# royshil/SfM-Toy-Library

Measured on NVIDIA H100. Metric: BA residual+Jacobian evals/sec, higher is better.
Workload: dtype f64

## Files before the change

sfm-toy-library_b200/csrc/ba.cu:

```cuda
#include "common.cuh"
#include "ba_math.cuh"
#include "chol.cuh"
#include <algorithm>
#include <chrono>
#include <cmath>
#include <cstdlib>

namespace {

constexpr int PT_THREADS = 128;
constexpr int PTB = 18;
constexpr int CAM_THREADS = 128;

struct LMState {
    double radius, decrease_factor, x_cost, x_norm, gmax, initial_cost;
    double msg_a, msg_b;
    double last_rho;
    int cur, iter, invalid_steps, new_point;
    int status;
    int termination_type;
    int num_successful, num_unsuccessful;
    int passes;
};
enum { LM_RUNNING = 0, LM_EVAL_FAILED = 1, LM_GRADIENT_TOL = 2, LM_MAX_TIME = 3, LM_MAX_ITER = 4, LM_MIN_RADIUS = 5, LM_INVALID_STEPS = 6,
       LM_PARAMETER_TOL = 7, LM_FUNCTION_TOL = 8 };

struct BAView {
    int nc, np, nobs, maxk;
    const LMState* st;
    double* cf2[2]; double* pts2[2]; CamDerived* camd2[2];
    const float2* obs_xy; const int32_t* obs_cam; const int32_t* pt_off;
    const int32_t* cm_off; const float2* cm_xy; const int32_t* cm_pt;
    const double* cams; const double* pts; const double* focal;
    const CamDerived* camd;
    const double* scale_cf; const double* scale_pt;
    double* ptblk;
    double* Zbuf;
    double* Sblk; double* Scf; double* Sff; double* rhs; double* gcf; double* dcf; double* sums;
    unsigned long long* gmax_pt_bits;
    int* fail;
    double min_diag, max_diag;
    double* part4;
    unsigned* counters;
};

__device__ __forceinline__ bool last_block_sum4(double* __restrict__ part4, unsigned* __restrict__ counter, const double (&mine)[4], double (&out)[4]) {
    __shared__ bool last_s;
    if (threadIdx.x == 0) {
#pragma unroll
        for (int q = 0; q < 4; ++q) part4[4 * (size_t)blockIdx.x + q] = mine[q];
        __threadfence();
        last_s = atomicInc(counter, gridDim.x - 1) == gridDim.x - 1;
    }
    __syncthreads();
    if (!last_s || threadIdx.x >= 32) return false;
    __threadfence();
    double acc[4] = {0.0, 0.0, 0.0, 0.0};
    for (unsigned b = threadIdx.x; b < gridDim.x; b += 32) {
#pragma unroll
        for (int q = 0; q < 4; ++q) acc[q] += __ldcg(part4 + 4 * (size_t)b + q);
    }
#pragma unroll
    for (int q = 0; q < 4; ++q) {
#pragma unroll
        for (int o = 16; o > 0; o >>= 1) acc[q] += __shfl_xor_sync(0xffffffffu, acc[q], o);
        out[q] = acc[q];
    }
    return true;
}

struct LMX { const double* focal; const double* pts; const CamDerived* camd; bool run; };
__device__ __forceinline__ LMX lm_x(const BAView& v) {
    LMX x; x.focal = v.focal; x.pts = v.pts; x.camd = v.camd; x.run = true;
    if (v.st) {
        x.run = v.st->status == LM_RUNNING;
        const int cur = v.st->cur;
        x.focal = v.cf2[cur] + 6 * v.nc; x.pts = v.pts2[cur]; x.camd = v.camd2[cur];
    }
    return x;
}

__device__ __forceinline__ void red_add(double* p, double v) {
    asm volatile("red.global.add.f64 [%0], %1;" ::"l"(p), "d"(v) : "memory");
}
__device__ __forceinline__ double clampd(double v, double lo, double hi) { return fmin(fmax(v, lo), hi); }
__device__ __forceinline__ size_t blk_index(int i, int j, int nb) {
    return (size_t)i * nb - (size_t)i * (i - 1) / 2 + (j - i);
}

template <int G>
__device__ __forceinline__ double group_sum(double v, unsigned mask) {
#pragma unroll
    for (int o = G / 2; o > 0; o >>= 1) v += __shfl_xor_sync(mask, v, o);
    return v;
}
__device__ __forceinline__ double warp_sum(double v) {
#pragma unroll
    for (int o = 16; o > 0; o >>= 1) v += __shfl_xor_sync(0xffffffffu, v, o);
    return v;
}
__device__ __forceinline__ double warp_max(double v) {
#pragma unroll
    for (int o = 16; o > 0; o >>= 1) v = fmax(v, __shfl_xor_sync(0xffffffffu, v, o));
    return v;
}

struct ObsJ { double r[2], Jc[12], Jp[6], Jf[2]; };
__device__ __forceinline__ void eval_scaled(const CamDerived& d, const double* X, double f, float2 xy,
                                            const double* sc , const double* sp , double sf, ObsJ& o) {
    obs_eval(d, X, f, (double)xy.x, (double)xy.y, o.r, o.Jc, o.Jp, o.Jf);
#pragma unroll
    for (int a = 0; a < 6; ++a) { o.Jc[a] *= sc[a]; o.Jc[6 + a] *= sc[a]; }
#pragma unroll
    for (int a = 0; a < 3; ++a) { o.Jp[a] *= sp[a]; o.Jp[3 + a] *= sp[a]; }
    o.Jf[0] *= sf; o.Jf[1] *= sf;
}

__global__ void cam_derive_kernel(const double* __restrict__ cams, int nc, CamDerived* __restrict__ out) {
    const int c = blockIdx.x * blockDim.x + threadIdx.x;
    if (c < nc) { CamDerived d; cam_derive(cams + 6 * c, d); out[c] = d; }
}

template <int G>
__global__ void __launch_bounds__(PT_THREADS) ba_point_norm_kernel(BAView v, double* __restrict__ scale_pt_out) {
    const int lane = threadIdx.x & 31, gl = lane % G;
    const unsigned gmask = G == 32 ? 0xffffffffu : (((1u << G) - 1u) << ((lane / G) * G));
    const int groups_per_block = PT_THREADS / G;
    const double f = *v.focal;
    for (int p = blockIdx.x * groups_per_block + threadIdx.x / G; p < v.np; p += gridDim.x * groups_per_block) {
        const int o0 = v.pt_off[p], k = v.pt_off[p + 1] - o0;
        const double X[3] = {v.pts[3 * p], v.pts[3 * p + 1], v.pts[3 * p + 2]};
        double n0 = 0, n1 = 0, n2 = 0;
        for (int j = gl; j < k; j += G) {
            const int o = o0 + j;
            double r[2], Jc[12], Jp[6], Jf[2];
            const float2 xy = v.obs_xy[o];
            obs_eval(v.camd[v.obs_cam[o]], X, f, (double)xy.x, (double)xy.y, r, Jc, Jp, Jf);
            n0 += Jp[0] * Jp[0] + Jp[3] * Jp[3]; n1 += Jp[1] * Jp[1] + Jp[4] * Jp[4]; n2 += Jp[2] * Jp[2] + Jp[5] * Jp[5];
        }
        n0 = group_sum<G>(n0, gmask); n1 = group_sum<G>(n1, gmask); n2 = group_sum<G>(n2, gmask);
        if (gl == 0) {
            scale_pt_out[3 * p] = 1.0 / (1.0 + sqrt(n0)); scale_pt_out[3 * p + 1] = 1.0 / (1.0 + sqrt(n1));
            scale_pt_out[3 * p + 2] = 1.0 / (1.0 + sqrt(n2));
        }
    }
}

__global__ void __launch_bounds__(CAM_THREADS) ba_camera_norm_kernel(BAView v, double* __restrict__ colnorm_cf) {
    const int c = blockIdx.y;
    const int begin = v.cm_off[c], end = v.cm_off[c + 1];
    const CamDerived d = v.camd[c];
    const double f = *v.focal;
    double n[7] = {0, 0, 0, 0, 0, 0, 0};
    for (int i = begin + blockIdx.x * CAM_THREADS + threadIdx.x; i < end; i += gridDim.x * CAM_THREADS) {
        const int p = v.cm_pt[i];
        const double X[3] = {v.pts[3 * p], v.pts[3 * p + 1], v.pts[3 * p + 2]};
        double r[2], Jc[12], Jp[6], Jf[2];
        const float2 xy = v.cm_xy[i];
        obs_eval(d, X, f, (double)xy.x, (double)xy.y, r, Jc, Jp, Jf);
#pragma unroll
        for (int a = 0; a < 6; ++a) n[a] += Jc[a] * Jc[a] + Jc[6 + a] * Jc[6 + a];
        n[6] += Jf[0] * Jf[0] + Jf[1] * Jf[1];
    }
    __shared__ double red[CAM_THREADS / 32][7];
#pragma unroll
    for (int a = 0; a < 7; ++a) { const double s = warp_sum(n[a]); if ((threadIdx.x & 31) == 0) red[threadIdx.x >> 5][a] = s; }
    __syncthreads();
    if (threadIdx.x < 7) {
        double s = 0;
        for (int w = 0; w < CAM_THREADS / 32; ++w) s += red[w][threadIdx.x];
        if (s != 0.0) red_add(threadIdx.x < 6 ? colnorm_cf + 6 * c + threadIdx.x : colnorm_cf + 6 * v.nc, s);
    }
}

__global__ void scale_from_norm_kernel(const double* __restrict__ colnorm, int n, double* __restrict__ scale) {
    const int i = blockIdx.x * blockDim.x + threadIdx.x;
    if (i < n) scale[i] = 1.0 / (1.0 + sqrt(colnorm[i]));
}
__global__ void fill_kernel(double* __restrict__ p, size_t n, double v) {
    const size_t i = (size_t)blockIdx.x * blockDim.x + threadIdx.x;
    if (i < n) p[i] = v;
}

template <int G, bool GATHER>
__global__ void __launch_bounds__(PT_THREADS, 3) ba_point_kernel(BAView v, double inv_radius) {
    const LMX x = lm_x(v);
    if (!x.run) return;
    if (v.st) inv_radius = 1.0 / v.st->radius;
    extern __shared__ __align__(16) unsigned char smem_raw[];
    __shared__ __align__(16) double zstage[GATHER ? PT_THREADS / 32 : 1][GATHER ? 32 * 18 : 2];
    constexpr int GB = PT_THREADS / G, GW = 32 / G;
    const int maxk = v.maxk;
    double* Zall = reinterpret_cast<double*>(smem_raw);
    int* camall = reinterpret_cast<int*>(Zall + (size_t)GB * maxk * 18);
    unsigned short* pair_tab = reinterpret_cast<unsigned short*>(camall + GB * maxk);
    if (!GATHER) {
        for (int j = 1 + threadIdx.x / 32; j < maxk; j += PT_THREADS / 32)
            for (int i = threadIdx.x & 31; i < j; i += 32) pair_tab[j * (j - 1) / 2 + i] = (unsigned short)(i | (j << 8));
        __syncthreads();
    }

    const int lane = threadIdx.x & 31, warp = threadIdx.x >> 5, gl = lane % G, gi = lane / G;
    const unsigned gmask = G == 32 ? 0xffffffffu : (((1u << G) - 1u) << (gi * G));
    const int group_in_block = warp * GW + gi;
    double* Zg = GATHER ? nullptr : Zall + (size_t)group_in_block * maxk * 18;
    int* camg = GATHER ? nullptr : camall + group_in_block * maxk;
    const double f = *x.focal, sf = v.scale_cf[6 * v.nc];
    const int nb = v.nc;

    double acc_cost = 0, acc_xn = 0, acc_sff = 0, acc_rf = 0, acc_gmax = 0;
    const int np_round = (v.np + GB - 1) / GB * GB;
    for (int base = blockIdx.x * GB; base < np_round; base += gridDim.x * GB) {
        const int p = base + group_in_block;
        const bool active = p < v.np;
        int o0 = 0, k = 0;
        double X[3] = {0, 0, 0}, sp[3] = {1, 1, 1};
        {
            const int pn = p + gridDim.x * GB;
            if (pn < v.np && gl == 0) {
                const int on = v.pt_off[pn];
                asm volatile("prefetch.global.L2 [%0];" :: "l"(v.obs_cam + on)); asm volatile("prefetch.global.L2 [%0];" :: "l"(v.obs_xy + on));
                asm volatile("prefetch.global.L2 [%0];" :: "l"(x.pts + 3 * (size_t)pn)); asm volatile("prefetch.global.L2 [%0];" :: "l"(v.scale_pt + 3 * (size_t)pn));
            }
        }
        if (active) {
            o0 = v.pt_off[p]; k = v.pt_off[p + 1] - o0;
            X[0] = x.pts[3 * p]; X[1] = x.pts[3 * p + 1]; X[2] = x.pts[3 * p + 2];
            sp[0] = v.scale_pt[3 * p]; sp[1] = v.scale_pt[3 * p + 1]; sp[2] = v.scale_pt[3 * p + 2];
        }
        double U[6] = {0, 0, 0, 0, 0, 0}, g[3] = {0, 0, 0}, wf[3] = {0, 0, 0}, cost = 0;
        double Wreg[18];
        for (int j = gl; j < k; j += G) {
            const int o = o0 + j, c = v.obs_cam[o];
            ObsJ J;
            eval_scaled(x.camd[c], X, f, v.obs_xy[o], v.scale_cf + 6 * c, sp, sf, J);
            const double* e = J.Jp;
            U[0] += e[0] * e[0] + e[3] * e[3]; U[1] += e[0] * e[1] + e[3] * e[4]; U[2] += e[0] * e[2] + e[3] * e[5];
            U[3] += e[1] * e[1] + e[4] * e[4]; U[4] += e[1] * e[2] + e[4] * e[5]; U[5] += e[2] * e[2] + e[5] * e[5];
#pragma unroll
            for (int a = 0; a < 3; ++a) { g[a] += e[a] * J.r[0] + e[3 + a] * J.r[1]; wf[a] += e[a] * J.Jf[0] + e[3 + a] * J.Jf[1]; }
            cost += J.r[0] * J.r[0] + J.r[1] * J.r[1];
            if (GATHER && j == gl) {
#pragma unroll
                for (int a = 0; a < 6; ++a)
#pragma unroll
                    for (int b = 0; b < 3; ++b) Wreg[a * 3 + b] = J.Jc[a] * e[b] + J.Jc[6 + a] * e[3 + b];
            } else {
                double* W = GATHER ? v.Zbuf + (size_t)o * 18 : Zg + j * 18;
#pragma unroll
                for (int a = 0; a < 6; ++a)
#pragma unroll
                    for (int b = 0; b < 3; ++b) W[a * 3 + b] = J.Jc[a] * e[b] + J.Jc[6 + a] * e[3 + b];
            }
            if (!GATHER) camg[j] = c;
        }
#pragma unroll
        for (int a = 0; a < 6; ++a) U[a] = group_sum<G>(U[a], gmask);
#pragma unroll
        for (int a = 0; a < 3; ++a) { g[a] = group_sum<G>(g[a], gmask); wf[a] = group_sum<G>(wf[a], gmask); }
        cost = group_sum<G>(cost, gmask);

        const double udiag[3] = {U[0], U[3], U[5]};
        U[0] += clampd(U[0], v.min_diag, v.max_diag) * inv_radius;
        U[3] += clampd(U[3], v.min_diag, v.max_diag) * inv_radius;
        U[5] += clampd(U[5], v.min_diag, v.max_diag) * inv_radius;
        double M[6] = {0, 0, 0, 0, 0, 0};
        const bool ok = chol3_inverse(U, M);
        if (!ok) { M[0] = M[1] = M[2] = M[3] = M[4] = M[5] = 0.0; }
        const double zg[3] = {M[0] * g[0], M[1] * g[0] + M[2] * g[1], M[3] * g[0] + M[4] * g[1] + M[5] * g[2]};
        const double zf[3] = {M[0] * wf[0], M[1] * wf[0] + M[2] * wf[1], M[3] * wf[0] + M[4] * wf[1] + M[5] * wf[2]};
        if (active) {
            const double blk[PTB] = {M[0], M[1], M[2], M[3], M[4], M[5], zg[0], zg[1], zg[2], zf[0], zf[1], zf[2], g[0], g[1], g[2], udiag[0], udiag[1], udiag[2]};
#pragma unroll
            for (int q = 0; q < PTB; ++q) if ((q % G) == gl) v.ptblk[(size_t)p * PTB + q] = blk[q];
            if (gl == 0) {
                if (!ok && k > 0) atomicAdd(v.fail, 1);
                acc_cost += cost;
                acc_xn += X[0] * X[0] + X[1] * X[1] + X[2] * X[2];
                acc_sff += zf[0] * zf[0] + zf[1] * zf[1] + zf[2] * zf[2];
                acc_rf += zf[0] * zg[0] + zf[1] * zg[1] + zf[2] * zg[2];
                acc_gmax = fmax(acc_gmax, fmax(fabs(g[0] / sp[0]), fmax(fabs(g[1] / sp[1]), fabs(g[2] / sp[2]))));
            }
        }
        const bool stage = GATHER && v.maxk <= G;
        int o_first = 0, o_end = 0;
        if (stage) {
            const int p_first = base + warp * GW;
            o_first = p_first < v.np ? v.pt_off[p_first] : 0; o_end = p_first < v.np ? v.pt_off[min(p_first + GW, v.np)] : 0;
        }
        if (GATHER && gl < k) {
            double2* dst = stage ? reinterpret_cast<double2*>(zstage[warp] + (size_t)(o0 + gl - o_first) * 18)
                                 : reinterpret_cast<double2*>(v.Zbuf + (size_t)(o0 + gl) * 18);
#pragma unroll
            for (int a = 0; a < 6; a += 2) {
                double z[6];
#pragma unroll
                for (int h = 0; h < 2; ++h) {
                    const double w0 = Wreg[(a + h) * 3], w1 = Wreg[(a + h) * 3 + 1], w2 = Wreg[(a + h) * 3 + 2];
                    z[3 * h] = w0 * M[0]; z[3 * h + 1] = w0 * M[1] + w1 * M[2]; z[3 * h + 2] = w0 * M[3] + w1 * M[4] + w2 * M[5];
                }
                dst[a / 2 * 3] = make_double2(z[0], z[1]); dst[a / 2 * 3 + 1] = make_double2(z[2], z[3]); dst[a / 2 * 3 + 2] = make_double2(z[4], z[5]);
            }
        }
        if (stage) {
            __syncwarp();
            const double2* src = reinterpret_cast<const double2*>(zstage[warp]);
            double2* out = reinterpret_cast<double2*>(v.Zbuf + (size_t)o_first * 18);
            for (int i = lane; i < (o_end - o_first) * 9; i += 32) out[i] = src[i];
            __syncwarp();
        }
        for (int j = gl + (GATHER ? G : 0); j < k; j += G) {
            double* W = GATHER ? v.Zbuf + (size_t)(o0 + j) * 18 : Zg + j * 18;
#pragma unroll
            for (int a = 0; a < 6; ++a) {
                const double w0 = W[a * 3], w1 = W[a * 3 + 1], w2 = W[a * 3 + 2];
                W[a * 3] = w0 * M[0]; W[a * 3 + 1] = w0 * M[1] + w1 * M[2]; W[a * 3 + 2] = w0 * M[3] + w1 * M[4] + w2 * M[5];
            }
        }
        if (GATHER) continue;
        __syncwarp();
#pragma unroll 1
        for (int gs = 0; gs < GW; ++gs) {
            const int kk = __shfl_sync(0xffffffffu, k, gs * G);
            const double* Zs = Zall + (size_t)(warp * GW + gs) * maxk * 18;
            const int* cs = camall + (warp * GW + gs) * maxk;
            const int total = kk * (kk - 1) / 2 * 36;
            for (int e = lane; e < total; e += 32) {
                const int pr = e / 36, ab = e - pr * 36, a = ab / 6, b = ab - a * 6;
                const unsigned ij = pair_tab[pr];
                const int i = ij & 0xff, j = ij >> 8;
                const double* zi = Zs + i * 18 + a * 3; const double* zj = Zs + j * 18 + b * 3;
                const double val = zi[0] * zj[0] + zi[1] * zj[1] + zi[2] * zj[2];
                red_add(v.Sblk + blk_index(cs[i], cs[j], nb) * 36 + ab, -val);
            }
        }
        __syncwarp();
    }
    __shared__ double sred[PT_THREADS / 32][5];
    const double c0 = warp_sum(acc_cost), c1 = warp_sum(acc_xn), c2 = warp_sum(acc_sff), c3 = warp_sum(acc_rf), c4 = warp_max(acc_gmax);
    if (lane == 0) { sred[warp][0] = c0; sred[warp][1] = c1; sred[warp][2] = c2; sred[warp][3] = c3; sred[warp][4] = c4; }
    __syncthreads();
    double t[4] = {0, 0, 0, 0};
    if (threadIdx.x == 0) {
        double t4 = 0;
        for (int w = 0; w < PT_THREADS / 32; ++w) { t[0] += sred[w][0]; t[1] += sred[w][1]; t[2] += sred[w][2]; t[3] += sred[w][3]; t4 = fmax(t4, sred[w][4]); }
        atomicMax(v.gmax_pt_bits, (unsigned long long)__double_as_longlong(t4));
        if (!GATHER) {
            red_add(v.sums + 0, t[0]); red_add(v.sums + 1, t[1]);
            red_add(v.Sff, -t[2]); red_add(v.rhs + 6 * v.nc, -t[3]);
        }
    }
    if (GATHER) {
        double tot[4];
        if (last_block_sum4(v.part4, v.counters + 0, t, tot) && threadIdx.x == 0) {
            v.sums[0] = tot[0]; v.sums[1] = tot[1]; *v.Sff = -tot[2]; v.rhs[6 * v.nc] = -tot[3];
        }
    }
}

__device__ __forceinline__ void dmma_m8n8k4(double& c0, double& c1, double a, double b) {
    asm volatile("mma.sync.aligned.m8n8k4.row.col.f64.f64.f64.f64 {%0,%1}, {%2}, {%3}, {%0,%1};" : "+d"(c0), "+d"(c1) : "d"(a), "d"(b));
}

constexpr int CAM_REC = 64;
template <bool DET, bool NORM_ONLY>
__global__ void __launch_bounds__(CAM_THREADS) ba_camera_kernel(BAView v, int per_cta, double* __restrict__ cam_part) {
    const LMX x = lm_x(v);
    if (!x.run) return;
    const int start = blockIdx.x * per_cta, stop = min(v.nobs, start + per_cta);
    if (start >= stop) return;
    int c = 0;
    {
        int lo = 0, hi = v.nc - 1;
        while (lo < hi) { const int mid = (lo + hi + 1) >> 1; if (v.cm_off[mid] <= start) lo = mid; else hi = mid - 1; }
        c = lo;
    }
    const double f = *x.focal, sf = NORM_ONLY ? 1.0 : v.scale_cf[6 * v.nc];
    __shared__ double red[CAM_THREADS / 32][48];
    const int lane = threadIdx.x & 31, warp = threadIdx.x >> 5;
    for (; c < v.nc && v.cm_off[c] < stop; ++c) {
    const int begin = max(start, v.cm_off[c]), end = min(stop, v.cm_off[c + 1]);
    if (begin >= end) continue;
    const CamDerived d = x.camd[c];
    double sc[6];
#pragma unroll
    for (int a = 0; a < 6; ++a) sc[a] = NORM_ONLY ? 1.0 : v.scale_cf[6 * c + a];
    double A[21], Cf[6], R[6], Gd[6], D[6], ff = 0, gf = 0;
#pragma unroll
    for (int a = 0; a < 21; ++a) A[a] = 0;
#pragma unroll
    for (int a = 0; a < 6; ++a) { Cf[a] = 0; R[a] = 0; Gd[a] = 0; D[a] = 0; }
    for (int i = begin + threadIdx.x; i < end; i += CAM_THREADS) {
        const int p = v.cm_pt[i];
        const double X[3] = {x.pts[3 * p], x.pts[3 * p + 1], x.pts[3 * p + 2]};
        ObsJ J;
        if (NORM_ONLY) {
            const double one[3] = {1.0, 1.0, 1.0};
            eval_scaled(d, X, f, v.cm_xy[i], sc, one, 1.0, J);
            ff += J.Jf[0] * J.Jf[0] + J.Jf[1] * J.Jf[1];
#pragma unroll
            for (int a = 0; a < 6; ++a) D[a] += J.Jc[a] * J.Jc[a] + J.Jc[6 + a] * J.Jc[6 + a];
            continue;
        }
        const double sp[3] = {v.scale_pt[3 * p], v.scale_pt[3 * p + 1], v.scale_pt[3 * p + 2]};
        const double* pb = v.ptblk + (size_t)p * PTB;
        const double M[6] = {pb[0], pb[1], pb[2], pb[3], pb[4], pb[5]};
        const double zg[3] = {pb[6], pb[7], pb[8]}, zf[3] = {pb[9], pb[10], pb[11]};
        eval_scaled(d, X, f, v.cm_xy[i], sc, sp, sf, J);
        ff += J.Jf[0] * J.Jf[0] + J.Jf[1] * J.Jf[1];
        gf += J.Jf[0] * J.r[0] + J.Jf[1] * J.r[1];
        double Z[6][3];
#pragma unroll
        for (int a = 0; a < 6; ++a) {
            const double w0 = J.Jc[a] * J.Jp[0] + J.Jc[6 + a] * J.Jp[3], w1 = J.Jc[a] * J.Jp[1] + J.Jc[6 + a] * J.Jp[4],
                         w2 = J.Jc[a] * J.Jp[2] + J.Jc[6 + a] * J.Jp[5];
            Z[a][0] = w0 * M[0]; Z[a][1] = w0 * M[1] + w1 * M[2]; Z[a][2] = w0 * M[3] + w1 * M[4] + w2 * M[5];
            const double jr = J.Jc[a] * J.r[0] + J.Jc[6 + a] * J.r[1];
            Gd[a] += jr;
            R[a] += jr - (Z[a][0] * zg[0] + Z[a][1] * zg[1] + Z[a][2] * zg[2]);
            Cf[a] += J.Jc[a] * J.Jf[0] + J.Jc[6 + a] * J.Jf[1] - (Z[a][0] * zf[0] + Z[a][1] * zf[1] + Z[a][2] * zf[2]);
            D[a] += J.Jc[a] * J.Jc[a] + J.Jc[6 + a] * J.Jc[6 + a];
        }
        int q = 0;
#pragma unroll
        for (int a = 0; a < 6; ++a)
#pragma unroll
            for (int b = a; b < 6; ++b, ++q)
                A[q] += J.Jc[a] * J.Jc[b] + J.Jc[6 + a] * J.Jc[6 + b] - (Z[a][0] * Z[b][0] + Z[a][1] * Z[b][1] + Z[a][2] * Z[b][2]);
    }
#pragma unroll
    for (int a = 0; a < 21; ++a) { const double s = warp_sum(A[a]); if (lane == 0) red[warp][a] = s; }
#pragma unroll
    for (int a = 0; a < 6; ++a) {
        const double s0 = warp_sum(Cf[a]), s1 = warp_sum(R[a]), s2 = warp_sum(Gd[a]), s3 = warp_sum(D[a]);
        if (lane == 0) { red[warp][21 + a] = s0; red[warp][27 + a] = s1; red[warp][33 + a] = s2; red[warp][39 + a] = s3; }
    }
    { const double s0 = warp_sum(ff), s1 = warp_sum(gf); if (lane == 0) { red[warp][45] = s0; red[warp][46] = s1; } }
    __syncthreads();
    if (threadIdx.x < 47) {
        double s = 0;
        for (int w = 0; w < CAM_THREADS / 32; ++w) s += red[w][threadIdx.x];
        const int t = threadIdx.x, fidx = 6 * v.nc;
        if (DET) {
            double* rec = cam_part + (size_t)(blockIdx.x + c) * CAM_REC;
            if (t < 21) {
                int a = 0, rem = t; while (rem >= 6 - a) { rem -= 6 - a; ++a; } const int b = a + rem;
                rec[a * 6 + b] = s; rec[b * 6 + a] = s;
            } else rec[36 + (t - 21)] = s;
        } else if (t < 21) {
            int a = 0, rem = t; while (rem >= 6 - a) { rem -= 6 - a; ++a; } const int b = a + rem;
            double* blk = v.Sblk + blk_index(c, c, v.nc) * 36;
            red_add(blk + a * 6 + b, s);
            if (a != b) red_add(blk + b * 6 + a, s);
        } else if (t < 27) red_add(v.Scf + 6 * c + (t - 21), s);
        else if (t < 33) red_add(v.rhs + 6 * c + (t - 27), s);
        else if (t < 39) red_add(v.gcf + 6 * c + (t - 33), s);
        else if (t < 45) red_add(v.dcf + 6 * c + (t - 39), s);
        else if (t == 45) { red_add(v.Sff, s); red_add(v.dcf + fidx, s); }
        else { red_add(v.rhs + fidx, s); red_add(v.gcf + fidx, s); }
    }
    __syncthreads();
    }
}

#include "ba_row.cuh"

__global__ void ba_assemble_kernel(const double* __restrict__ Sblk, const double* __restrict__ Scf, const double* __restrict__ Sff,
                                   const double* __restrict__ rhs, const double* __restrict__ dcf, int nc, int npad,
                                   double inv_radius, double min_diag, double max_diag, double* __restrict__ A, const LMState* __restrict__ st,
                                   unsigned* __restrict__ solve_counter) {
    if (st) { if (st->status != LM_RUNNING) return; inv_radius = 1.0 / st->radius; }
    if (solve_counter && blockIdx.x == 0 && blockIdx.y == 0 && threadIdx.x == 0) *solve_counter += 1u;
    const int n = 6 * nc + 1;
    const int c = blockIdx.x * blockDim.x + threadIdx.x, r = blockIdx.y;
    if (c >= npad || c > r) return;
    double val;
    if (r < n) {
        if (r == n - 1) val = (c == n - 1) ? *Sff : Scf[c];
        else {
            const int bi = r / 6, a = r - 6 * bi, bj = c / 6, b = c - 6 * bj;
            val = Sblk[blk_index(bj, bi, nc) * 36 + b * 6 + a];
        }
        if (r == c) val += clampd(dcf[r], min_diag, max_diag) * inv_radius;
    } else if (r == n) val = c < n ? rhs[c] : 0.0;
    else val = (r == c) ? 1.0 : 0.0;
    A[(size_t)r * npad + c] = val;
}

__global__ void __launch_bounds__(256) ba_cam_update_kernel(BAView v, double inv_radius, const double* x_cf, const double* __restrict__ y_cf,
                                                            const double* __restrict__ scale_cf, const double* __restrict__ gcf, int nc,
                                                            double* cand_cf, CamDerived* camd_c, double* __restrict__ locals,
                                                            double* __restrict__ post, const unsigned long long* __restrict__ gmax_pt_bits,
                                                            const int* __restrict__ fail) {
    if (v.st) {
        if (v.st->status != LM_RUNNING) return;
        const int cur = v.st->cur;
        x_cf = v.cf2[cur]; cand_cf = v.cf2[cur ^ 1]; camd_c = v.camd2[cur ^ 1];
        inv_radius = 1.0 / v.st->radius;
    }
    const int n = 6 * nc + 1;
    double dn = 0, xn = 0, cn = 0, gm = 0, mc = 0;
    for (int i = threadIdx.x; i < n; i += blockDim.x) {
        const double yi = y_cf[i], d = -yi * scale_cf[i], xv = x_cf[i], cv = xv + d;
        cand_cf[i] = cv;
        const double dd = xv - cv;
        dn += dd * dd; xn += xv * xv; cn += cv * cv;
        gm = fmax(gm, fabs(gcf[i] / scale_cf[i]));
        mc -= 0.5 * yi * (gcf[i] + clampd(v.dcf[i], v.min_diag, v.max_diag) * inv_radius * yi);
    }
    __shared__ double red[8][5];
    const double a = warp_sum(dn), b = warp_sum(xn), c = warp_sum(cn), g = warp_max(gm), m = warp_sum(mc);
    if ((threadIdx.x & 31) == 0) { red[threadIdx.x >> 5][0] = a; red[threadIdx.x >> 5][1] = b; red[threadIdx.x >> 5][2] = c; red[threadIdx.x >> 5][3] = g; red[threadIdx.x >> 5][4] = m; }
    __syncthreads();
    if (threadIdx.x == 0) {
        double s0 = 0, s1 = 0, s2 = 0, s3 = 0, s4 = 0;
        for (int w = 0; w < 8; ++w) { s0 += red[w][0]; s1 += red[w][1]; s2 += red[w][2]; s3 = fmax(s3, red[w][3]); s4 += red[w][4]; }
        locals[0] = s0; locals[1] = s1; locals[2] = s2; locals[3] = s3; locals[4] = s4;
        post[7] = __longlong_as_double((long long)*gmax_pt_bits);
        post[4] = (double)fail[0]; post[5] = (double)fail[1];
        post[0] = post[1] = post[2] = post[3] = post[6] = 0.0;
    }
    __syncthreads();
    for (int c2 = threadIdx.x; c2 < nc; c2 += blockDim.x) { CamDerived d; cam_derive(cand_cf + 6 * c2, d); camd_c[c2] = d; }
}

__global__ void ba_lm_control_kernel(LMState* __restrict__ st, const double* __restrict__ sums, const double* __restrict__ post,
                                     const double* __restrict__ locals, sfmb200_ba_options opt) {
    if (threadIdx.x != 0 || blockIdx.x != 0 || st->status != LM_RUNNING) return;
    LMState s = *st;
    ++s.passes;
    const double cost_x = 0.5 * sums[0], xn2_pts = sums[1];
    const double cand_cost_raw = 0.5 * post[0], model_acc = post[1] + locals[4], dn2_pts = post[2], cn2_pts = post[3];
    const double fail0 = post[4], fail1 = post[5], gmax_pt = post[7];
    const double dn2_cf = locals[0], xn2_cf = locals[1], cn2_cf = locals[2], gmax_cf = locals[3];
    auto stop = [&](int status, int type) { s.status = status; s.termination_type = type; *st = s; };
    if (s.new_point) {
        s.x_cost = cost_x; s.x_norm = sqrt(xn2_pts + xn2_cf); s.gmax = fmax(gmax_pt, gmax_cf);
        s.new_point = 0;
        if (s.iter == 0) {
            s.initial_cost = s.x_cost;
            if (!isfinite(s.x_cost)) return stop(LM_EVAL_FAILED, SFMB200_BA_FAILURE);
            if (s.gmax <= opt.gradient_tolerance) return stop(LM_GRADIENT_TOL, SFMB200_BA_CONVERGENCE);
            if (s.iter >= opt.max_num_iterations) return stop(LM_MAX_ITER, SFMB200_BA_NO_CONVERGENCE);
        }
    }
    if (s.gmax <= opt.gradient_tolerance) return stop(LM_GRADIENT_TOL, SFMB200_BA_CONVERGENCE);
    if (s.radius <= opt.min_trust_region_radius) return stop(LM_MIN_RADIUS, SFMB200_BA_CONVERGENCE);
    ++s.iter;
    const bool lin_ok = fail0 == 0.0 && fail1 == 0.0 && isfinite(model_acc) && isfinite(dn2_pts) && isfinite(dn2_cf);
    const double model_cost_change = -model_acc;
    bool decided = false;
    if (!lin_ok || !(model_cost_change > 0.0)) {
        s.num_unsuccessful++;
        if (++s.invalid_steps >= opt.max_num_consecutive_invalid_steps) return stop(LM_INVALID_STEPS, SFMB200_BA_FAILURE);
        s.radius /= s.decrease_factor; s.decrease_factor *= 2.0;
        decided = true;
    }
    if (!decided) {
        s.invalid_steps = 0;
        const double step_norm = sqrt(dn2_pts + dn2_cf);
        const double cand_cost = isfinite(cand_cost_raw) ? cand_cost_raw : 1.7976931348623157e308;
        if (step_norm <= opt.parameter_tolerance * (s.x_norm + opt.parameter_tolerance)) {
            s.msg_a = step_norm / (s.x_norm + opt.parameter_tolerance); s.msg_b = opt.parameter_tolerance;
            return stop(LM_PARAMETER_TOL, SFMB200_BA_CONVERGENCE);
        }
        const double cost_change = s.x_cost - cand_cost;
        if (fabs(cost_change) <= opt.function_tolerance * s.x_cost) {
            s.msg_a = fabs(cost_change) / s.x_cost; s.msg_b = opt.function_tolerance;
            return stop(LM_FUNCTION_TOL, SFMB200_BA_CONVERGENCE);
        }
        const double relative_decrease = cost_change / model_cost_change;
        s.last_rho = relative_decrease;
        if (relative_decrease > opt.min_relative_decrease) {
            s.cur ^= 1;
            s.x_norm = sqrt(cn2_pts + cn2_cf); s.new_point = 1;
            const double q = 2.0 * relative_decrease - 1.0;
            s.radius = fmin(opt.max_trust_region_radius, s.radius / fmax(1.0 / 3.0, 1.0 - q * q * q));
            s.decrease_factor = 2.0;
            s.num_successful++;
            s.x_cost = cand_cost;
        } else {
            s.radius /= s.decrease_factor; s.decrease_factor *= 2.0;
            s.num_unsuccessful++;
        }
    }
    if (s.iter >= opt.max_num_iterations) return stop(LM_MAX_ITER, SFMB200_BA_NO_CONVERGENCE);
    *st = s;
}

template <int G, bool CAMTAB>
__global__ void __launch_bounds__(PT_THREADS) ba_backsub_z_kernel(BAView v, double inv_radius, const double* __restrict__ y_cf, const double* cand_cf,
                                                                  const CamDerived* camd_c, double* pts_c, double* __restrict__ post) {
    extern __shared__ __align__(16) double camtab[];
    const LMX x = lm_x(v);
    if (!x.run) return;
    if (v.st) { const int nxt = v.st->cur ^ 1; cand_cf = v.cf2[nxt]; camd_c = v.camd2[nxt]; pts_c = v.pts2[nxt]; inv_radius = 1.0 / v.st->radius; }
    const int lane = threadIdx.x & 31, warp = threadIdx.x >> 5, gl = lane % G;
    const unsigned gmask = G == 32 ? 0xffffffffu : (((1u << G) - 1u) << ((lane / G) * G));
    constexpr int GB = PT_THREADS / G;
    const double yf = y_cf[6 * v.nc], fc = cand_cf[6 * v.nc];
    if (CAMTAB) {
        for (int i = threadIdx.x; i < v.nc * 18; i += PT_THREADS) {
            const int c = i / 18, q = i - 18 * c;
            camtab[i] = q < 12 ? reinterpret_cast<const double*>(camd_c + c)[q] : y_cf[6 * c + q - 12];
        }
        __syncthreads();
    }
    double acc_cc = 0, acc_m = 0, acc_dn = 0, acc_cn = 0;
    constexpr int GW = 32 / G;
    __shared__ __align__(16) double zstage[PT_THREADS / 32][32 * 18];
    const int np_round = (v.np + GB - 1) / GB * GB;
    int o0_next = 0, k_next = 0;
    { const int pn = blockIdx.x * GB + threadIdx.x / G; if (pn < v.np) { o0_next = v.pt_off[pn]; k_next = v.pt_off[pn + 1] - o0_next; } }
    for (int p0 = blockIdx.x * GB; p0 < np_round; p0 += gridDim.x * GB) {
        const int p = p0 + threadIdx.x / G;
        const bool active = p < v.np;
        const int o0 = o0_next, k = k_next;
        {
            const int pn = p + gridDim.x * GB;
            o0_next = 0; k_next = 0;
            if (pn < v.np) {
                o0_next = v.pt_off[pn]; k_next = v.pt_off[pn + 1] - o0_next;
                if (gl < k_next) {
                    const char* zr = reinterpret_cast<const char*>(v.Zbuf + (size_t)(o0_next + gl) * 18);
                    asm volatile("prefetch.global.L2 [%0];" :: "l"(zr)); asm volatile("prefetch.global.L2 [%0];" :: "l"(zr + 128));
                }
                if (gl == 0) {
                    asm volatile("prefetch.global.L2 [%0];" :: "l"(v.obs_cam + o0_next)); asm volatile("prefetch.global.L2 [%0];" :: "l"(v.obs_xy + o0_next));
                    asm volatile("prefetch.global.L2 [%0];" :: "l"(x.pts + 3 * (size_t)pn)); asm volatile("prefetch.global.L2 [%0];" :: "l"(v.scale_pt + 3 * (size_t)pn));
                    const char* pbn = reinterpret_cast<const char*>(v.ptblk + (size_t)pn * PTB);
                    asm volatile("prefetch.global.L2 [%0];" :: "l"(pbn)); asm volatile("prefetch.global.L2 [%0];" :: "l"(pbn + 128));
                }
            }
        }
        const bool stage = v.maxk <= G;
        int o_first = 0;
        if (stage) {
            o_first = __shfl_sync(0xffffffffu, o0, 0);
            const int o_end = (int)__reduce_max_sync(0xffffffffu, (unsigned)(o0 + k));
            __syncwarp();
            const double2* in = reinterpret_cast<const double2*>(v.Zbuf + (size_t)o_first * 18);
            double2* dstz = reinterpret_cast<double2*>(zstage[warp]);
            for (int i = lane; i < (o_end - o_first) * 9; i += 32) dstz[i] = in[i];
            __syncwarp();
        }
        double t[3] = {0, 0, 0};
        for (int j = gl; j < k; j += G) {
            const int o = o0 + j, c = v.obs_cam[o];
            const double2* z = stage ? reinterpret_cast<const double2*>(zstage[warp] + (size_t)(o - o_first) * 18)
                                     : reinterpret_cast<const double2*>(v.Zbuf + (size_t)o * 18);
#pragma unroll
            for (int a = 0; a < 6; a += 2) {
                const double2 z0 = z[a / 2 * 3], z1 = z[a / 2 * 3 + 1], z2 = z[a / 2 * 3 + 2];
                const double ya = CAMTAB ? camtab[18 * c + 12 + a] : y_cf[6 * c + a], yb = CAMTAB ? camtab[18 * c + 13 + a] : y_cf[6 * c + a + 1];
                t[0] += z0.x * ya + z1.y * yb; t[1] += z0.y * ya + z2.x * yb; t[2] += z1.x * ya + z2.y * yb;
            }
        }
#pragma unroll
        for (int a = 0; a < 3; ++a) t[a] = group_sum<G>(t[a], gmask);
        if (!active) continue;
        const double X[3] = {x.pts[3 * p], x.pts[3 * p + 1], x.pts[3 * p + 2]};
        const double sp[3] = {v.scale_pt[3 * p], v.scale_pt[3 * p + 1], v.scale_pt[3 * p + 2]};
        const double* pb = v.ptblk + (size_t)p * PTB;
        const double M[6] = {pb[0], pb[1], pb[2], pb[3], pb[4], pb[5]};
        const double u0 = pb[6] - t[0] - pb[9] * yf, u1 = pb[7] - t[1] - pb[10] * yf, u2 = pb[8] - t[2] - pb[11] * yf;
        const double yp[3] = {M[0] * u0 + M[1] * u1 + M[3] * u2, M[2] * u1 + M[4] * u2, M[5] * u2};
        const double Xc[3] = {X[0] - yp[0] * sp[0], X[1] - yp[1] * sp[1], X[2] - yp[2] * sp[2]};
        if (gl == 0) {
            pts_c[3 * p] = Xc[0]; pts_c[3 * p + 1] = Xc[1]; pts_c[3 * p + 2] = Xc[2];
            const double d0 = X[0] - Xc[0], d1 = X[1] - Xc[1], d2 = X[2] - Xc[2];
            acc_dn += d0 * d0 + d1 * d1 + d2 * d2;
            acc_cn += Xc[0] * Xc[0] + Xc[1] * Xc[1] + Xc[2] * Xc[2];
#pragma unroll
            for (int a = 0; a < 3; ++a) acc_m -= 0.5 * yp[a] * (pb[12 + a] + clampd(pb[15 + a], v.min_diag, v.max_diag) * inv_radius * yp[a]);
        }
        for (int j = gl; j < k; j += G) {
            const int o = o0 + j, c = v.obs_cam[o];
            const float2 xy = v.obs_xy[o];
            double rc[2];
            if (CAMTAB) {
                const double* ct = camtab + 18 * c;
                const double p0 = ct[0] * Xc[0] + ct[1] * Xc[1] + ct[2] * Xc[2] + ct[9];
                const double p1 = ct[3] * Xc[0] + ct[4] * Xc[1] + ct[5] * Xc[2] + ct[10];
                const double p2 = ct[6] * Xc[0] + ct[7] * Xc[1] + ct[8] * Xc[2] + ct[11];
                const double iz = 1.0 / p2;
                rc[0] = fc * (p0 * iz) - (double)xy.x; rc[1] = fc * (p1 * iz) - (double)xy.y;
            } else obs_residual(camd_c[c], Xc, fc, (double)xy.x, (double)xy.y, rc);
            acc_cc += rc[0] * rc[0] + rc[1] * rc[1];
        }
    }
    __shared__ double sred[PT_THREADS / 32][4];
    const double c0 = warp_sum(acc_cc), c1 = warp_sum(acc_m), c2 = warp_sum(acc_dn), c3 = warp_sum(acc_cn);
    if (lane == 0) { sred[warp][0] = c0; sred[warp][1] = c1; sred[warp][2] = c2; sred[warp][3] = c3; }
    __syncthreads();
    double t[4] = {0, 0, 0, 0};
    if (threadIdx.x == 0) for (int w = 0; w < PT_THREADS / 32; ++w) { t[0] += sred[w][0]; t[1] += sred[w][1]; t[2] += sred[w][2]; t[3] += sred[w][3]; }
    double tot[4];
    if (last_block_sum4(v.part4, v.counters + 1, t, tot) && threadIdx.x == 0) { post[0] = tot[0]; post[1] = tot[1]; post[2] = tot[2]; post[3] = tot[3]; }
}

struct BacksubCam {
    CamDerived d;
    double Rc[9], tc[3];
    double ys[6];
};
template <int G, bool CAMTAB>
__global__ void __launch_bounds__(PT_THREADS) ba_backsub_eval_kernel(BAView v, double inv_radius, const double* __restrict__ y_cf, const double* cand_cf,
                                                                     const CamDerived* camd_c, double* pts_c, double* __restrict__ post) {
    extern __shared__ __align__(16) unsigned char bs_smem[];
    BacksubCam* camtab = reinterpret_cast<BacksubCam*>(bs_smem);
    const LMX x = lm_x(v);
    if (!x.run) return;
    if (v.st) { const int nxt = v.st->cur ^ 1; cand_cf = v.cf2[nxt]; camd_c = v.camd2[nxt]; pts_c = v.pts2[nxt]; inv_radius = 1.0 / v.st->radius; }
    const int lane = threadIdx.x & 31, warp = threadIdx.x >> 5, gl = lane % G;
    const unsigned gmask = G == 32 ? 0xffffffffu : (((1u << G) - 1u) << ((lane / G) * G));
    constexpr int GB = PT_THREADS / G;
    const double f = *x.focal, yfs = v.scale_cf[6 * v.nc] * y_cf[6 * v.nc], fc = cand_cf[6 * v.nc];
    if (CAMTAB) {
        constexpr int CD = sizeof(CamDerived) / 8, CT = sizeof(BacksubCam) / 8;
        double* tab = reinterpret_cast<double*>(bs_smem);
        for (int i = threadIdx.x; i < v.nc * CT; i += PT_THREADS) {
            const int c = i / CT, q = i - CT * c;
            tab[i] = q < CD ? reinterpret_cast<const double*>(x.camd + c)[q]
                   : q < CD + 12 ? reinterpret_cast<const double*>(camd_c + c)[q - CD]
                   : v.scale_cf[6 * c + q - CD - 12] * y_cf[6 * c + q - CD - 12];
        }
        __syncthreads();
    }
    double acc_cc = 0, acc_m = 0, acc_dn = 0, acc_cn = 0;
    const int np_round = (v.np + GB - 1) / GB * GB;
    int o0_next = 0, k_next = 0;
// ... 1020 lines not shown
```

Baseline: 1.672 billion.

## Stream W blocks through staging buffer, share camera data, prefetch point indices

In the point kernel, the per-observation W blocks are now written as double2 straight to the warp's shared staging buffer (or to Zbuf) instead of holding the first one in 18 registers. They are then scaled by M in place in a single unified loop, which drops the Wreg array to cut register pressure. In the camera kernel, camera-derived data and scales are loaded once into shared memory per camera, and the cm_pt indices are software-pipelined two iterations ahead to hide index-load latency. The costs are an extra __syncthreads per camera, a reload of W from memory, and a new dependence on shared memory and staging-buffer traffic.

Result: no change. 1.678 billion, median of 6 (+0.3%).

```diff
diff --git a/sfm-toy-library_b200/csrc/ba.cu b/sfm-toy-library_b200/csrc/ba.cu
--- a/sfm-toy-library_b200/csrc/ba.cu
+++ b/sfm-toy-library_b200/csrc/ba.cu
@@ -228,8 +228,17 @@
             X[0] = x.pts[3 * p]; X[1] = x.pts[3 * p + 1]; X[2] = x.pts[3 * p + 2];
             sp[0] = v.scale_pt[3 * p]; sp[1] = v.scale_pt[3 * p + 1]; sp[2] = v.scale_pt[3 * p + 2];
         }
+        const bool stage = GATHER && v.maxk <= G;
+        int o_first = 0, o_end = 0;
+        if (stage) {
+            const int p_first = base + warp * GW;
+            o_first = p_first < v.np ? v.pt_off[p_first] : 0; o_end = p_first < v.np ? v.pt_off[min(p_first + GW, v.np)] : 0;
+        }
+        auto zrec = [&](int j) {
+            return reinterpret_cast<double2*>(GATHER ? (stage ? zstage[warp] + (size_t)(o0 + j - o_first) * 18 : v.Zbuf + (size_t)(o0 + j) * 18)
+                                                     : Zg + j * 18);
+        };
         double U[6] = {0, 0, 0, 0, 0, 0}, g[3] = {0, 0, 0}, wf[3] = {0, 0, 0}, cost = 0;
-        double Wreg[18];
         for (int j = gl; j < k; j += G) {
             const int o = o0 + j, c = v.obs_cam[o];
             ObsJ J;
@@ -240,17 +249,15 @@
 #pragma unroll
             for (int a = 0; a < 3; ++a) { g[a] += e[a] * J.r[0] + e[3 + a] * J.r[1]; wf[a] += e[a] * J.Jf[0] + e[3 + a] * J.Jf[1]; }
             cost += J.r[0] * J.r[0] + J.r[1] * J.r[1];
-            if (GATHER && j == gl) {
-#pragma unroll
-                for (int a = 0; a < 6; ++a)
-#pragma unroll
-                    for (int b = 0; b < 3; ++b) Wreg[a * 3 + b] = J.Jc[a] * e[b] + J.Jc[6 + a] * e[3 + b];
-            } else {
-                double* W = GATHER ? v.Zbuf + (size_t)o * 18 : Zg + j * 18;
-#pragma unroll
-                for (int a = 0; a < 6; ++a)
-#pragma unroll
-                    for (int b = 0; b < 3; ++b) W[a * 3 + b] = J.Jc[a] * e[b] + J.Jc[6 + a] * e[3 + b];
+            double2* W = zrec(j);
+#pragma unroll
+            for (int a = 0; a < 6; a += 2) {
+                double w[6];
+#pragma unroll
+                for (int h = 0; h < 2; ++h)
+#pragma unroll
+                    for (int b = 0; b < 3; ++b) w[3 * h + b] = J.Jc[a + h] * e[b] + J.Jc[6 + a + h] * e[3 + b];
+                W[a / 2 * 3] = make_double2(w[0], w[1]); W[a / 2 * 3 + 1] = make_double2(w[2], w[3]); W[a / 2 * 3 + 2] = make_double2(w[4], w[5]);
             }
             if (!GATHER) camg[j] = c;
         }
@@ -282,24 +289,19 @@
                 acc_gmax = fmax(acc_gmax, fmax(fabs(g[0] / sp[0]), fmax(fabs(g[1] / sp[1]), fabs(g[2] / sp[2]))));
             }
         }
-        const bool stage = GATHER && v.maxk <= G;
-        int o_first = 0, o_end = 0;
-        if (stage) {
-            const int p_first = base + warp * GW;
-            o_first = p_first < v.np ? v.pt_off[p_first] : 0; o_end = p_first < v.np ? v.pt_off[min(p_first + GW, v.np)] : 0;
-        }
-        if (GATHER && gl < k) {
-            double2* dst = stage ? reinterpret_cast<double2*>(zstage[warp] + (size_t)(o0 + gl - o_first) * 18)
-                                 : reinterpret_cast<double2*>(v.Zbuf + (size_t)(o0 + gl) * 18);
+        for (int j = gl; j < k; j += G) {
+            double2* W = zrec(j);
 #pragma unroll
             for (int a = 0; a < 6; a += 2) {
+                const double2 p0 = W[a / 2 * 3], p1 = W[a / 2 * 3 + 1], p2 = W[a / 2 * 3 + 2];
+                const double w[6] = {p0.x, p0.y, p1.x, p1.y, p2.x, p2.y};
                 double z[6];
 #pragma unroll
                 for (int h = 0; h < 2; ++h) {
-                    const double w0 = Wreg[(a + h) * 3], w1 = Wreg[(a + h) * 3 + 1], w2 = Wreg[(a + h) * 3 + 2];
+                    const double w0 = w[3 * h], w1 = w[3 * h + 1], w2 = w[3 * h + 2];
                     z[3 * h] = w0 * M[0]; z[3 * h + 1] = w0 * M[1] + w1 * M[2]; z[3 * h + 2] = w0 * M[3] + w1 * M[4] + w2 * M[5];
                 }
-                dst[a / 2 * 3] = make_double2(z[0], z[1]); dst[a / 2 * 3 + 1] = make_double2(z[2], z[3]); dst[a / 2 * 3 + 2] = make_double2(z[4], z[5]);
+                W[a / 2 * 3] = make_double2(z[0], z[1]); W[a / 2 * 3 + 1] = make_double2(z[2], z[3]); W[a / 2 * 3 + 2] = make_double2(z[4], z[5]);
             }
         }
         if (stage) {
@@ -308,14 +310,6 @@
             double2* out = reinterpret_cast<double2*>(v.Zbuf + (size_t)o_first * 18);
             for (int i = lane; i < (o_end - o_first) * 9; i += 32) out[i] = src[i];
             __syncwarp();
-        }
-        for (int j = gl + (GATHER ? G : 0); j < k; j += G) {
-            double* W = GATHER ? v.Zbuf + (size_t)(o0 + j) * 18 : Zg + j * 18;
-#pragma unroll
-            for (int a = 0; a < 6; ++a) {
-                const double w0 = W[a * 3], w1 = W[a * 3 + 1], w2 = W[a * 3 + 2];
-                W[a * 3] = w0 * M[0]; W[a * 3 + 1] = w0 * M[1] + w1 * M[2]; W[a * 3 + 2] = w0 * M[3] + w1 * M[4] + w2 * M[5];
-            }
         }
         if (GATHER) continue;
         __syncwarp();
@@ -377,21 +371,27 @@
     }
     const double f = *x.focal, sf = NORM_ONLY ? 1.0 : v.scale_cf[6 * v.nc];
     __shared__ double red[CAM_THREADS / 32][48];
+    __shared__ CamDerived cam_s;
+    __shared__ double sc_s[6];
     const int lane = threadIdx.x & 31, warp = threadIdx.x >> 5;
     for (; c < v.nc && v.cm_off[c] < stop; ++c) {
     const int begin = max(start, v.cm_off[c]), end = min(stop, v.cm_off[c + 1]);
     if (begin >= end) continue;
-    const CamDerived d = x.camd[c];
-    double sc[6];
-#pragma unroll
-    for (int a = 0; a < 6; ++a) sc[a] = NORM_ONLY ? 1.0 : v.scale_cf[6 * c + a];
+    if (threadIdx.x == 0) cam_s = x.camd[c];
+    if (threadIdx.x < 6) sc_s[threadIdx.x] = NORM_ONLY ? 1.0 : v.scale_cf[6 * c + threadIdx.x];
+    __syncthreads();
+    const CamDerived& d = cam_s;
+    const double* sc = sc_s;
     double A[21], Cf[6], R[6], Gd[6], D[6], ff = 0, gf = 0;
 #pragma unroll
     for (int a = 0; a < 21; ++a) A[a] = 0;
 #pragma unroll
     for (int a = 0; a < 6; ++a) { Cf[a] = 0; R[a] = 0; Gd[a] = 0; D[a] = 0; }
+    int p = begin + threadIdx.x < end ? v.cm_pt[begin + threadIdx.x] : 0;
+    int pn = begin + threadIdx.x + CAM_THREADS < end ? v.cm_pt[begin + threadIdx.x + CAM_THREADS] : 0;
     for (int i = begin + threadIdx.x; i < end; i += CAM_THREADS) {
-        const int p = v.cm_pt[i];
+        asm volatile("" ::: "memory");
+        const int pnn = i + 2 * CAM_THREADS < end ? v.cm_pt[i + 2 * CAM_THREADS] : 0;
         const double X[3] = {x.pts[3 * p], x.pts[3 * p + 1], x.pts[3 * p + 2]};
         ObsJ J;
         if (NORM_ONLY) {
@@ -400,6 +400,7 @@
             ff += J.Jf[0] * J.Jf[0] + J.Jf[1] * J.Jf[1];
 #pragma unroll
             for (int a = 0; a < 6; ++a) D[a] += J.Jc[a] * J.Jc[a] + J.Jc[6 + a] * J.Jc[6 + a];
+            p = pn; pn = pnn;
             continue;
         }
         const double sp[3] = {v.scale_pt[3 * p], v.scale_pt[3 * p + 1], v.scale_pt[3 * p + 2]};
@@ -427,6 +428,7 @@
 #pragma unroll
             for (int b = a; b < 6; ++b, ++q)
                 A[q] += J.Jc[a] * J.Jc[b] + J.Jc[6 + a] * J.Jc[6 + b] - (Z[a][0] * Z[b][0] + Z[a][1] * Z[b][1] + Z[a][2] * Z[b][2]);
+        p = pn; pn = pnn;
     }
 #pragma unroll
     for (int a = 0; a < 21; ++a) { const double s = warp_sum(A[a]); if (lane == 0) red[warp][a] = s; }
```
